# mynameisfiber/baton

Measured on NVIDIA H100. Metric: federated local samples/sec (whole box), ResNet-18 FedAvg, synthetic non-IID 32x32 shards, higher is better.
Workload: dtype bf16

## Files before the change

### baton_b200/csrc/bindings.cpp

```cpp
#include <ATen/cuda/CUDAContext.h>
#include <c10/cuda/CUDAGuard.h>
#include <torch/extension.h>

#include <optional>
#include <vector>

#include "launch.h"

namespace {

inline cudaStream_t cur_stream() { return at::cuda::getCurrentCUDAStream().stream(); }
inline void check(int rc, const char* what) {
  TORCH_CHECK(rc == 0, "baton_b200::", what, " failed with code ", rc,
              rc > 0 ? std::string(" (") + cudaGetErrorString(static_cast<cudaError_t>(rc)) + ")" : std::string());
}
inline const void* cptr(const at::Tensor& t) { return t.data_ptr(); }
inline void* ptr(at::Tensor& t) { return t.data_ptr(); }
template <class T>
inline T* opt_ptr(const std::optional<at::Tensor>& t) {
  return (t.has_value() && t->defined()) ? reinterpret_cast<T*>(t->data_ptr()) : nullptr;
}
#define CHECK_CUDA(x) TORCH_CHECK((x).is_cuda(), #x " must be a CUDA tensor")

inline std::optional<B200SgdEpilogue> sgd_epilogue(const std::optional<at::Tensor>& theta,
// ... 118 lines not shown
  return true;
}

bool conv_igemm_fwd(const at::Tensor& x, const at::Tensor& w, at::Tensor y, int64_t kh, int64_t kw, int64_t stride,
                    int64_t pad, int64_t ho, int64_t wo, int64_t cluster_k, int64_t force_bn,
                    const std::optional<at::Tensor>& col_stats) {
  CHECK_CUDA(x); CHECK_CUDA(w); CHECK_CUDA(y);
  TORCH_CHECK(x.scalar_type() == at::kBFloat16 && w.scalar_type() == at::kBFloat16 && y.scalar_type() == at::kBFloat16 &&
              x.dim() == 4 && x.is_contiguous() && w.is_contiguous() && y.is_contiguous());
  const c10::cuda::CUDAGuard guard(x.device());
  const int rc = b200_conv_igemm_fwd(cptr(x), cptr(w), ptr(y), static_cast<int>(x.size(0)), static_cast<int>(x.size(1)),
                                     static_cast<int>(x.size(2)), static_cast<int>(x.size(3)), static_cast<int>(w.size(0)),
                                     static_cast<int>(kh), static_cast<int>(kw), static_cast<int>(stride),
                                     static_cast<int>(pad), static_cast<int>(ho), static_cast<int>(wo),
                                     static_cast<int>(cluster_k), static_cast<int>(force_bn), opt_ptr<float>(col_stats),
                                     cur_stream());
  if (rc == -2) return false;
  check(rc, "conv_igemm_fwd");
  return true;
}
bool conv_igemm_dgrad(const at::Tensor& dy, const at::Tensor& w, at::Tensor dx, int64_t kh, int64_t kw, int64_t pad,
                      int64_t cluster_k, int64_t force_bn) {
  CHECK_CUDA(dy); CHECK_CUDA(w); CHECK_CUDA(dx);
  TORCH_CHECK(dy.scalar_type() == at::kBFloat16 && w.scalar_type() == at::kBFloat16 && dx.scalar_type() == at::kBFloat16 &&
              dy.dim() == 4 && dx.dim() == 4 && dy.is_contiguous() && w.is_contiguous() && dx.is_contiguous());
  const c10::cuda::CUDAGuard guard(dy.device());
  const int rc = b200_conv_igemm_dgrad(cptr(dy), cptr(w), ptr(dx), static_cast<int>(dx.size(0)), static_cast<int>(dx.size(1)),
                                       static_cast<int>(dx.size(2)), static_cast<int>(dx.size(3)), static_cast<int>(dy.size(3)),
                                       static_cast<int>(kh), static_cast<int>(kw), static_cast<int>(pad),
                                       static_cast<int>(dy.size(1)), static_cast<int>(dy.size(2)),
                                       static_cast<int>(cluster_k), static_cast<int>(force_bn), cur_stream());
  if (rc == -2) return false;
  check(rc, "conv_igemm_dgrad");
  return true;
}
bool conv_igemm_wgrad(const at::Tensor& dy, const at::Tensor& x, at::Tensor dw, int64_t cout, int64_t kh, int64_t kw,
                      int64_t stride, int64_t pad, int64_t ho, int64_t wo, int64_t split_k, int64_t force_bn,
                      const std::optional<at::Tensor>& sgd_theta, const std::optional<at::Tensor>& sgd_theta_bf16,
                      const std::optional<at::Tensor>& sgd_mom, const std::optional<at::Tensor>& sgd_hyper,
                      bool sgd_nesterov) {
  CHECK_CUDA(dy); CHECK_CUDA(x); CHECK_CUDA(dw);
  TORCH_CHECK(x.scalar_type() == at::kBFloat16 && dy.scalar_type() == at::kBFloat16 && dw.scalar_type() == at::kFloat &&
              x.dim() == 4 && x.is_contiguous() && dy.is_contiguous());
  const c10::cuda::CUDAGuard guard(x.device());
  const std::optional<B200SgdEpilogue> sgd = sgd_epilogue(sgd_theta, sgd_theta_bf16, sgd_mom, sgd_hyper, sgd_nesterov);
  const int rc = b200_conv_igemm_wgrad(cptr(dy), cptr(x), dw.data_ptr<float>(), static_cast<int>(x.size(0)),
                                       static_cast<int>(x.size(1)), static_cast<int>(x.size(2)), static_cast<int>(x.size(3)),
                                       static_cast<int>(cout), static_cast<int>(kh), static_cast<int>(kw),
                                       static_cast<int>(stride), static_cast<int>(pad), static_cast<int>(ho),
                                       static_cast<int>(wo), static_cast<int>(split_k), static_cast<int>(force_bn),
                                       sgd ? &*sgd : nullptr, cur_stream());
  if (rc == -2 || rc == B200_SGD_EPILOGUE_DECLINED) return false;
  check(rc, "conv_igemm_wgrad");
  return true;
}

void gemm_fp8(const at::Tensor& a, const at::Tensor& b, at::Tensor d, const std::optional<at::Tensor>& bias,
              const std::optional<at::Tensor>& sfa, const std::optional<at::Tensor>& sfb, int64_t M, int64_t N, int64_t K,
              int64_t lda, int64_t ldb, int64_t ldd, int64_t act, int64_t split_k, bool accumulate, double alpha) {
  CHECK_CUDA(a); CHECK_CUDA(b); CHECK_CUDA(d);
  TORCH_CHECK(a.element_size() == 1 && b.element_size() == 1, "gemm_fp8 operands must be 1-byte (e4m3)");
  const c10::cuda::CUDAGuard guard(a.device());
  check(b200_gemm_fp8(cptr(a), cptr(b), ptr(d), opt_ptr<const float>(bias), opt_ptr<const void>(sfa),
                      opt_ptr<const void>(sfb), M, N, K, lda, ldb, ldd, d.scalar_type() == at::kFloat, act, split_k,
                      accumulate, static_cast<float>(alpha), cur_stream()),
        "gemm_fp8");
// ... 405 lines not shown
                                       dw.data_ptr<float>(), opt_ptr<float>(db), loss_acc.data_ptr<float>(),
                                       opt_ptr<float>(logits_out), static_cast<int>(x.size(0)), static_cast<int>(x.size(1)),
                                       static_cast<int>(w.size(0)), static_cast<float>(grad_scale), cur_stream());
  if (rc == -2) return false;
  check(rc, "linear_xent_head");
  return true;
}
void mse(const at::Tensor& pred, const at::Tensor& target, const std::optional<at::Tensor>& dpred, at::Tensor loss_acc,
         double grad_scale) {
  CHECK_CUDA(pred);
  TORCH_CHECK(target.scalar_type() == at::kFloat && target.numel() == pred.numel());
  const c10::cuda::CUDAGuard guard(pred.device());
  const int in32 = pred.scalar_type() == at::kFloat;
  const int out32 = dpred.has_value() && dpred->defined() && dpred->scalar_type() == at::kFloat;
  check(b200_mse(pred.data_ptr(), in32, target.data_ptr<float>(), opt_ptr<void>(dpred), out32,
                 loss_acc.data_ptr<float>(), pred.numel(), static_cast<float>(grad_scale), cur_stream()),
        "mse");
}

}

PYBIND11_MODULE(TORCH_EXTENSION_NAME, m) {
  m.doc() = "baton_b200 sm_90a kernels";
  m.attr("MAX_RANKS") = B200_MAX_RANKS;
  m.def("gemm", &gemm);
  m.def("trace_set", &trace_set);
  m.def("attention_fwd", &attention_fwd);
  m.def("attention_bwd", &attention_bwd);
  m.def("bn_bwd_cluster", &bn_bwd_cluster);
  m.def("im2col_tma_probe", &im2col_tma_probe);
  m.def("conv_igemm_fwd", &conv_igemm_fwd);
  m.def("conv_igemm_wgrad", &conv_igemm_wgrad);
  m.def("conv_igemm_dgrad", &conv_igemm_dgrad);
  m.def("gemm_batched", &gemm_batched);
  m.def("gemm_fp8", &gemm_fp8);
  m.def("quant_mx_rows", &quant_mx_rows);
  m.def("quant_mx_cols", &quant_mx_cols);
  m.def("dequant_mx", &dequant_mx);
  m.def("fused_sgd", &fused_sgd);
  m.def("fused_sgd_segments", &fused_sgd_segments);
  m.def("weighted_sum", &weighted_sum);
  m.def("fold_client", &fold_client);
  m.def("cast", &cast);
  m.def("gather_rows", &gather_rows);
  m.def("colsum", &colsum);
  m.def("add_bf16", &add_bf16);
  m.def("relu_bwd", &relu_bwd);
  m.def("gelu", &gelu);
  m.def("gelu_bwd", &gelu_bwd);
  m.def("pad_rows", &pad_rows);
  m.def("embedding_bwd", &embedding_bwd);
  m.def("fedavg_allreduce", &fedavg_allreduce);
  m.def("flag_barrier", &flag_barrier);
  m.def("im2col", &im2col);
  m.def("col2im", &col2im);
  m.def("maxpool", &maxpool);
  m.def("maxpool_bwd", &maxpool_bwd);
  m.def("avgpool", &avgpool);
  m.def("avgpool_bwd", &avgpool_bwd);
  m.def("bn_stats", &bn_stats);
  m.def("bn_apply", &bn_apply);
  m.def("bn_bwd_reduce", &bn_bwd_reduce);
  m.def("bn_bwd_apply", &bn_bwd_apply);
  m.def("bn_relu_maxpool", &bn_relu_maxpool);
  m.def("bn_maxpool_bwd", &bn_maxpool_bwd);
  m.def("layernorm_fwd", &layernorm_fwd);
// ... 8 lines not shown
```

### baton_b200/csrc/gemm_wgmma.cu

```cuda
#define B200_TU_TAG 1
#include "ptx.cuh"
#include "launch.h"
#include "pdl.cuh"
#include "sgd.cuh"

namespace b200 {

constexpr int BM = 128;
constexpr int BK = 64;
constexpr int WG_K = 16;
constexpr int GEMM_THREADS = 384;
constexpr int CONSUMER_WARPS = 8;
constexpr int CONSUMER_THREADS = 32 * CONSUMER_WARPS;
constexpr int MAX_STAGES = 8;

struct GemmParams {
  int M, N, K;
  void* D;
  long long ldd;
  const float* bias;
  int out_fp32;
  int act;
  float* col_stats;
  int a_mn, b_mn;
  int k_tiles_per_split;
  int atomic_out;
  int cluster_k;
  int stages;
  const uint32_t* tile_flags;
  uint32_t flag_epoch;
  long long flag_elem_off;
  int flag_tile_elems;
  long long flag_bias_off;
  long long ldb;
  float alpha;
  int batched, batch_inner;
  int batch_count;
  long long d_outer, d_inner;
  int conv_ho, conv_wo;
  int conv_stride, conv_pad;
  int conv_kw;
  int conv_cin;
  int conv_taps;
  int conv_ncol;
  const uint32_t* flag_epoch_ptr;
  const float* sgd_hyper = nullptr;
  float* sgd_theta = nullptr;
  __nv_bfloat16* sgd_wb = nullptr;
  float* sgd_mom = nullptr;
  int sgd_nesterov = 0;
};

__device__ __forceinline__ void wait_arrival_flags(const uint32_t* flags, long long e0, long long e1, int granule,
                                                   uint32_t need) {
  for (long long t = e0 / granule; t <= e1 / granule; ++t) {
    unsigned long long spins = 0;
    while (static_cast<int32_t>(ld_acquire_sys(flags + t) - need) < 0) {
      if (++spins > (1ull << 26)) break;
    }
  }
}

template <int BN>
struct SmemLayout {
  static constexpr int A_BYTES = BM * BK * 2;
  static constexpr int B_BYTES = BN * BK * 2;
  static constexpr int STAGE_BYTES = A_BYTES + B_BYTES;
  static constexpr int PART_PITCH = BN + 4;
  static constexpr int PART_BYTES = BM * PART_PITCH * 4;
};

__device__ __forceinline__ float apply_act(float v, int act) {
  if (act == 1) return fmaxf(v, 0.f);
  if (act == 2) {
    const float k0 = 0.7978845608028654f, k1 = 0.044715f;
    float t = tanhf(k0 * (v + k1 * v * v * v));
    return 0.5f * v * (1.f + t);
  }
  return v;
}

__device__ __forceinline__ uint32_t cluster_ctarank() {
  uint32_t r;
// ... 172 lines not shown
      }
    }
  }
}

template <int BN>
__device__ __forceinline__ void consume_ktiles(float (&acc)[BN / 2], uint8_t* smem, int stages, uint64_t* full_bar,
                                               uint64_t* empty_bar, int& s, uint32_t& ph, int num_kt, int a_mn,
                                               int b_mn, int g) {
  using L = SmemLayout<BN>;
#pragma unroll
  for (int j = 0; j < BN / 2; ++j) acc[j] = 0.f;
  int prev = -1;
  for (int i = 0; i < num_kt; ++i) {
    mbar_wait(&full_bar[s], ph);
    const uint32_t sa = smem_u32(smem + s * L::STAGE_BYTES) + g * 8192;
    const uint32_t sb = smem_u32(smem + s * L::STAGE_BYTES + L::A_BYTES);
    wgmma_fence();
#pragma unroll
    for (int k = 0; k < BK / WG_K; ++k) {
      const uint64_t ad = a_mn ? gmma_desc_sw128(sa + k * 2048, 8192, 1024) : gmma_desc_sw128(sa + k * 32, 16, 1024);
      const uint64_t bd = b_mn ? gmma_desc_sw128(sb + k * 2048, 8192, 1024) : gmma_desc_sw128(sb + k * 32, 16, 1024);
      wgmma_bf16<BN>(acc, ad, bd, 1u, a_mn, b_mn);
    }
    wgmma_commit();
    wgmma_wait<1>();
    if (prev >= 0 && lane_id() == 0) mbar_arrive(&empty_bar[prev]);
    prev = s;
    if (++s == stages) { s = 0; ph ^= 1; }
  }
  wgmma_wait<0>();
  wgmma_fence_operands(acc);
  if (prev >= 0 && lane_id() == 0) mbar_arrive(&empty_bar[prev]);
}

template <int BN, int STAGES, int CONV = 0, bool SGD = false>
__global__ void __launch_bounds__(GEMM_THREADS, 1)
gemm_bf16_fixed_kernel(const __grid_constant__ CUtensorMap tmA, const __grid_constant__ CUtensorMap tmB,
                         const GemmParams p) {
  using L = SmemLayout<BN>;
  static_assert(STAGES * L::STAGE_BYTES >= L::PART_BYTES, "the drained ring must hold the fp32 accumulator tile");
  extern __shared__ __align__(1024) uint8_t smem_raw[];
  uint8_t* smem = reinterpret_cast<uint8_t*>((reinterpret_cast<uintptr_t>(smem_raw) + 1023) & ~uintptr_t(1023));
  uint64_t* full_bar = reinterpret_cast<uint64_t*>(smem + STAGES * L::STAGE_BYTES);
  uint64_t* empty_bar = full_bar + STAGES;
  float* cstat = reinterpret_cast<float*>(empty_bar + STAGES);

  griddep_launch_dependents();
  const int warp = threadIdx.x >> 5;
  const int m0 = blockIdx.y * BM;
  const int n0 = blockIdx.x * BN;
  const int k_tiles_total = (p.K + BK - 1) / BK;
  const int bz_outer = p.batched ? static_cast<int>(blockIdx.z) / p.batch_inner : 0;
  const int bz_inner = p.batched ? static_cast<int>(blockIdx.z) % p.batch_inner : 0;
  const int kt_begin = p.batched ? 0 : blockIdx.z * p.k_tiles_per_split;
  int kt_end = kt_begin + p.k_tiles_per_split;
  if (kt_end > k_tiles_total) kt_end = k_tiles_total;
  const int num_kt = kt_end - kt_begin;

  if (warp == 0 && elect_one()) {
    tma_prefetch_desc(&tmA);
    tma_prefetch_desc(&tmB);
    for (int s = 0; s < STAGES; ++s) {
      mbar_init(&full_bar[s], 1);
      mbar_init(&empty_bar[s], CONSUMER_WARPS);
    }
    fence_barrier_init();
  }
  __syncthreads();
  griddep_wait();

  if (warp == 0) {
    if (elect_one()) {
      if (p.tile_flags != nullptr) {
        const int rows_here = (p.N - n0) < BN ? (p.N - n0) : BN;
        const uint32_t need = p.flag_epoch_ptr != nullptr ? *reinterpret_cast<const volatile uint32_t*>(p.flag_epoch_ptr)
                                                          : p.flag_epoch;
        wait_arrival_flags(p.tile_flags, p.flag_elem_off + static_cast<long long>(n0) * p.ldb,
                           p.flag_elem_off + static_cast<long long>(n0 + rows_here) * p.ldb - 1, p.flag_tile_elems, need);
        if (p.flag_bias_off >= 0)
          wait_arrival_flags(p.tile_flags, p.flag_bias_off + n0, p.flag_bias_off + n0 + rows_here - 1,
                             p.flag_tile_elems, need);
        fence_proxy_async_all();
      }
      TRACE_POINT();
      for (int i = 0; i < num_kt; ++i) {
        const int s = i % STAGES;
        const uint32_t ph = (i / STAGES) & 1;
        mbar_wait(&empty_bar[s], ph ^ 1);
        uint8_t* sa = smem + s * L::STAGE_BYTES;
        uint8_t* sb = sa + L::A_BYTES;
        const int k0 = (kt_begin + i) * BK;
        if constexpr (CONV == 2) {
          const int live = (p.N - n0 + 63) / 64 < BN / 64 ? (p.N - n0 + 63) / 64 : BN / 64;
          mbar_expect_tx(&full_bar[s], L::A_BYTES + live * 8192);
        } else {
          mbar_expect_tx(&full_bar[s], L::STAGE_BYTES);
        }
        if (p.batched) {
          if (!p.a_mn) {
            tma_load_4d(sa, &tmA, &full_bar[s], k0, m0, bz_inner, bz_outer);
          } else {
#pragma unroll
            for (int j = 0; j < BM / 64; ++j)
              tma_load_4d(sa + j * 8192, &tmA, &full_bar[s], m0 + j * 64, k0, bz_inner, bz_outer);
          }
          if (!p.b_mn) {
            tma_load_4d(sb, &tmB, &full_bar[s], k0, n0, bz_inner, bz_outer);
          } else {
#pragma unroll
            for (int j = 0; j < BN / 64; ++j)
              tma_load_4d(sb + j * 8192, &tmB, &full_bar[s], n0 + j * 64, k0, bz_inner, bz_outer);
          }
        } else {
        if constexpr (CONV == 1 || CONV == 3) {
          const int kt = kt_begin + i;
          const int cblocks = p.conv_cin >> 6;
          const int tap = kt / cblocks, cb = kt - tap * cblocks;
          const int fr = tap / p.conv_kw, fs = tap - fr * p.conv_kw;
          const int q0 = m0 % p.conv_wo, t0 = m0 / p.conv_wo;
          tma_load_im2col_4d(sa, &tmA, &full_bar[s], cb * 64, q0 * p.conv_stride - p.conv_pad,
                             (t0 % p.conv_ho) * p.conv_stride - p.conv_pad, t0 / p.conv_ho, fs, fr);
        } else if (!p.a_mn) {
          tma_load_2d(sa, &tmA, &full_bar[s], k0, m0);
        } else {
#pragma unroll
          for (int j = 0; j < BM / 64; ++j)
            tma_load_2d(sa + j * 8192, &tmA, &full_bar[s], m0 + j * 64, k0);
        }
        if constexpr (CONV == 2) {
          const int q0 = k0 % p.conv_wo, t0 = k0 / p.conv_wo;
          const int w0 = q0 * p.conv_stride - p.conv_pad, h0 = (t0 % p.conv_ho) * p.conv_stride - p.conv_pad;
          const int img = t0 / p.conv_ho;
#pragma unroll
          for (int j = 0; j < BN / 64; ++j) {
            const int col = n0 + j * 64;
            if (col < p.N) {
              const int tap = col / p.conv_cin, c = col - tap * p.conv_cin;
              const int fr = tap / p.conv_kw, fs = tap - fr * p.conv_kw;
              tma_load_im2col_4d(sb + j * 8192, &tmB, &full_bar[s], c, w0, h0, img, fs, fr);
            }
          }
        } else if constexpr (CONV == 3) {
          const int kt = kt_begin + i;
          const int cblocks = p.conv_cin >> 6;
          const int tap = kt / cblocks, cb = kt - tap * cblocks;
          const int wcol = (p.conv_taps - 1 - tap) * p.conv_ncol + n0;
#pragma unroll
          for (int j = 0; j < BN / 64; ++j) tma_load_2d(sb + j * 8192, &tmB, &full_bar[s], wcol + j * 64, cb * 64);
        } else if (!p.b_mn) {
          tma_load_2d(sb, &tmB, &full_bar[s], k0, n0);
        } else {
#pragma unroll
          for (int j = 0; j < BN / 64; ++j) tma_load_2d(sb + j * 8192, &tmB, &full_bar[s], n0 + j * 64, k0);
        }
        }
      }
    }
  } else if (warp >= 4) {
    const int ew = warp - 4;
    float acc[BN / 2];
    int s = 0;
    uint32_t ph = 0;
    consume_ktiles<BN>(acc, smem, STAGES, full_bar, empty_bar, s, ph, num_kt, p.a_mn, p.b_mn, ew >> 2);
    if (threadIdx.x == 128) TRACE_POINT();
    named_bar_sync(1, CONSUMER_THREADS);
    float* part = reinterpret_cast<float*>(smem);
    wg_store_acc<BN>(acc, part, L::PART_PITCH, 64 * (ew >> 2));
    named_bar_sync(1, CONSUMER_THREADS);
    const int q = ew & 3;
    constexpr int NCHUNK = BN / 32;
    const int c_begin = (ew < 4 ? 0 : (NCHUNK + 1) / 2) * 32, c_end = (ew < 4 ? (NCHUNK + 1) / 2 : NCHUNK) * 32;
    const int lrow = q * 32 + static_cast<int>(lane_id());
    const int row = m0 + lrow;
    const bool row_ok = row < p.M;
    const size_t elt = p.out_fp32 ? 4 : 2;
    uint8_t* drow = reinterpret_cast<uint8_t*>(p.D) +
                    (static_cast<size_t>(row) * p.ldd + static_cast<size_t>(bz_outer) * p.d_outer +
                     static_cast<size_t>(bz_inner) * p.d_inner) * elt;
    const bool vec_ok = ((reinterpret_cast<uintptr_t>(p.D) & 15) == 0) && ((p.ldd * elt) % 16 == 0);
    const bool sgd_vec = SGD && (p.ldd % 4 == 0) &&
                         ((reinterpret_cast<uintptr_t>(p.sgd_theta) | reinterpret_cast<uintptr_t>(p.sgd_mom)) & 15) == 0 &&
                         (reinterpret_cast<uintptr_t>(p.sgd_wb) & 7) == 0;
    float* sstat = cstat + q * 2 * BN;
    const bool want_stats = p.col_stats != nullptr;
#pragma unroll 1
    for (int c = c_begin; c < c_end; c += 32) {
      uint32_t r[32];
      acc_ld_row32(part + lrow * L::PART_PITCH + c, r);
      const int col0 = n0 + c;
      float v[32];
#pragma unroll
      for (int j = 0; j < 32; ++j) v[j] = __uint_as_float(r[j]);
      if (col0 >= p.N) {
        if (want_stats) { sstat[c + lane_id()] = 0.f; sstat[BN + c + lane_id()] = 0.f; }
        continue;
      }
      transform_chunk<32>(p, col0, v);
      if (want_stats) stage_col_stats(sstat, BN, c, v);
      if (!row_ok) continue;
      const bool full = (col0 + 32 <= p.N);
      if constexpr (SGD) {
        sgd_epilogue_chunk(p, static_cast<size_t>(row) * p.ldd + col0, col0, v, sgd_vec);
        continue;
      }
      if (p.atomic_out) {
        float* d = reinterpret_cast<float*>(drow) + col0;
        if (full && vec_ok) {
#pragma unroll
          for (int j = 0; j < 32; j += 4)
            asm volatile("red.global.add.v4.f32 [%0], {%1, %2, %3, %4};" ::"l"(d + j), "f"(v[j]), "f"(v[j + 1]),
// ... 735 lines not shown
      (reinterpret_cast<uintptr_t>(w) & 15) || (reinterpret_cast<uintptr_t>(dx) & 15))
    return -2;
  const int bn = clamp_bn(force_bn > 0 ? force_bn : (Cin > 64 ? 128 : 64));
  CUtensorMap ta, tb;
  int rc = b200_encode_map_im2col_bf16(&ta, dy, N, Ho, Wo, Cout, KH, KW, 1, padp, 64, BM);
  if (rc) return rc;
  rc = make_map(&tb, w, Cout, static_cast<long long>(KH) * KW * Cin, static_cast<long long>(KH) * KW * Cin, 64, BK);
  if (rc) return rc;
  const int k_tiles = K / BK;
  if (cluster_k != 1 && cluster_k != 2 && cluster_k != 4 && cluster_k != 8) return -5;
  while (cluster_k > 1 && (cluster_k - 1) * ((k_tiles + cluster_k - 1) / cluster_k) >= k_tiles) cluster_k >>= 1;
  const int per = (k_tiles + cluster_k - 1) / cluster_k;
  GemmParams p;
  p.M = static_cast<int>(M); p.N = Cin; p.K = K; p.D = dx; p.ldd = Cin; p.bias = nullptr; p.out_fp32 = 0; p.act = 0;
  p.a_mn = 0; p.b_mn = 1; p.k_tiles_per_split = per; p.cluster_k = cluster_k; p.atomic_out = 0;
  p.col_stats = nullptr;
  p.tile_flags = nullptr; p.flag_epoch = 0; p.alpha = 1.0f; p.flag_elem_off = 0; p.flag_tile_elems = 0;
  p.ldb = static_cast<long long>(KH) * KW * Cin;
  p.flag_bias_off = -1; p.flag_epoch_ptr = nullptr;
  p.batched = 0; p.batch_inner = 1; p.batch_count = 1; p.d_outer = 0; p.d_inner = 0;
  const int max_stages = bn == 128 ? 6 : 8;
  p.stages = per < max_stages ? (per < 2 ? 2 : per) : max_stages;
  p.conv_ho = H; p.conv_wo = W; p.conv_stride = 1; p.conv_pad = padp; p.conv_kw = KW; p.conv_cin = Cout;
  p.conv_taps = KH * KW; p.conv_ncol = Cin;
  dim3 grid((Cin + bn - 1) / bn, static_cast<unsigned>((M + BM - 1) / BM), cluster_k);
  if (cluster_k > 1) {
    if (bn == 128) return launch_cfg<128, 3>(ta, tb, p, grid, stream);
    return launch_cfg<64, 3>(ta, tb, p, grid, stream);
  }
  if (bn == 128) return launch_fixed<128, 6, 3>(ta, tb, p, grid, stream);
  return launch_fixed<64, 8, 3>(ta, tb, p, grid, stream);
}

extern "C" int b200_conv_igemm_wgrad(const void* dy, const void* x, float* dw, int N, int H, int W, int Cin, int Cout,
                                     int KH, int KW, int stride, int pad, int Ho, int Wo, int split_k, int force_bn,
                                     const B200SgdEpilogue* sgd, cudaStream_t stream) {
  using namespace b200;
  const long long Mp = static_cast<long long>(N) * Ho * Wo;
  const int Kc = KH * KW * Cin;
  if (Mp <= 0 || Cout <= 0) return 0;
  if (Cin % 64 != 0 || Cout % 8 != 0 || Mp > (1ll << 30) || (reinterpret_cast<uintptr_t>(x) & 15) ||
      (reinterpret_cast<uintptr_t>(dy) & 15) || (reinterpret_cast<uintptr_t>(dw) & 15))
    return -2;
  const int bn = clamp_bn(force_bn > 0 ? force_bn : (Kc > 64 ? 128 : 64));
  CUtensorMap ta, tb;
  int rc = make_map(&ta, dy, Mp, Cout, Cout, 64, BK);
  if (rc) return rc;
  rc = b200_encode_map_im2col_bf16(&tb, x, N, H, W, Cin, KH, KW, stride, pad, 64, 64);
  if (rc) return rc;
  const int k_tiles = static_cast<int>((Mp + BK - 1) / BK);
  if (split_k < 1) split_k = 1;
  if (split_k > k_tiles) split_k = k_tiles;
  const int per = (k_tiles + split_k - 1) / split_k;
  split_k = (k_tiles + per - 1) / per;
  if (sgd != nullptr && split_k != 1) return B200_SGD_EPILOGUE_DECLINED;
  GemmParams p;
  if (sgd != nullptr) set_sgd_epilogue(p, *sgd);
  p.M = Cout; p.N = Kc; p.K = static_cast<int>(Mp); p.D = dw; p.ldd = Kc; p.bias = nullptr; p.out_fp32 = 1; p.act = 0;
  p.a_mn = 1; p.b_mn = 1; p.k_tiles_per_split = per; p.cluster_k = 1; p.atomic_out = 1;
  p.col_stats = nullptr;
  p.tile_flags = nullptr; p.flag_epoch = 0; p.alpha = 1.0f; p.flag_elem_off = 0; p.flag_tile_elems = 0; p.ldb = Kc;
  p.flag_bias_off = -1; p.flag_epoch_ptr = nullptr;
  p.batched = 0; p.batch_inner = 1; p.batch_count = 1; p.d_outer = 0; p.d_inner = 0;
  p.stages = 4;
  p.conv_ho = Ho; p.conv_wo = Wo; p.conv_stride = stride; p.conv_pad = pad; p.conv_kw = KW; p.conv_cin = Cin;
  p.conv_taps = KH * KW; p.conv_ncol = Cin;
// ... 11 lines not shown
```

### baton_b200/csrc/launch.h

```cpp
#pragma once
#include <cuda_runtime.h>
#include <stdint.h>

#define B200_MAX_RANKS 16

extern "C" {

struct B200SgdEpilogue {
  float* theta;
  void* theta_bf16;
  float* mom;
  const float* hyper;
  int nesterov;
};
#define B200_SGD_EPILOGUE_DECLINED (-6)

int b200_gemm_bf16(const void* a, const void* b, void* d, const float* bias, int M, int N, int K, long long lda,
                   long long ldb, long long ldd, int a_mn, int b_mn, int out_fp32, int act, int split_k, int accumulate,
                   float alpha, const uint32_t* tile_flags, uint32_t flag_epoch, long long flag_elem_off, int flag_tile_elems,
                   long long flag_bias_off, int force_bn, float* col_stats, const uint32_t* flag_epoch_ptr,
                   const B200SgdEpilogue* sgd, cudaStream_t stream);
int b200_gemm_bf16_batched(const void* a, const void* b, void* d, int M, int N, int K, long long lda, long long ldb,
                           long long ldd, int a_mn, int b_mn, int out_fp32, int act, float alpha, int n_outer,
                           int n_inner, long long a_outer, long long a_inner, long long b_outer, long long b_inner,
                           long long d_outer, long long d_inner, int accumulate, cudaStream_t stream);
int b200_attention_fwd(const void* qkv, void* out, void* probs, int B, int S, int H, int dh, float scale,
                       cudaStream_t stream);
int b200_attention_bwd(const void* qkv, const void* dout, const void* probs, void* dqkv, int B, int S, int H, int dh,
                       float scale, cudaStream_t stream);
int b200_conv_igemm_fwd(const void* x, const void* w, void* y, int N, int H, int W, int Cin, int Cout, int KH, int KW,
                        int stride, int pad, int Ho, int Wo, int cluster_k, int force_bn, float* col_stats,
                        cudaStream_t stream);
int b200_conv_igemm_dgrad(const void* dy, const void* w, void* dx, int N, int H, int W, int Cin, int Cout, int KH, int KW,
                          int pad, int Ho, int Wo, int cluster_k, int force_bn, cudaStream_t stream);
int b200_conv_igemm_wgrad(const void* dy, const void* x, float* dw, int N, int H, int W, int Cin, int Cout, int KH, int KW,
                          int stride, int pad, int Ho, int Wo, int split_k, int force_bn, const B200SgdEpilogue* sgd,
                          cudaStream_t stream);
int b200_im2col_tma_probe(const void* x, void* col, int N, int H, int W, int C, int KH, int KW, int stride, int pad,
                          int Ho, int Wo, cudaStream_t stream);
int b200_gemm_fp8(const void* a, const void* b, void* d, const float* bias, const void* sfa, const void* sfb, int M, int N,
                  int K, long long lda, long long ldb, long long ldd, int out_fp32, int act, int split_k, int accumulate,
                  float alpha, cudaStream_t stream);
int b200_quant_mx_rows(const void* x, void* q, void* sf, long long R, int C, long long ld_in, int Cp, cudaStream_t stream);
int b200_quant_mx_cols(const void* x, void* q, void* sf, long long R, int C, long long ld_in, long long Rp,
                       cudaStream_t stream);
int b200_dequant_mx(const void* q, const void* sf, float* out, long long R, int C, int Cp, cudaStream_t stream);
int b200_gemm_simt(const void* a, const void* b, void* d, const float* bias, int M, int N, int K, long long lda,
                   long long ldb, long long ldd, int a_mn, int b_mn, int out_fp32, int act, int accumulate,
                   float alpha, cudaStream_t stream);

int b200_fused_sgd(float* w, float* g, float* mom, void* w_bf16, long long n, const float* hyper, int zero_grad,
                   int nesterov, const unsigned long long* wire_slot, const float* pack_global,
                   const float* pack_scale, long long n_pack, int wire_fp32, cudaStream_t stream);
int b200_fused_sgd_segments(float* w, float* g, float* mom, void* w_bf16, const long long* segments, int n_seg,
                            const float* hyper, int nesterov, cudaStream_t stream);
int b200_fold_client(float* acc, float* theta, const float* global_w, void* w_bf16, float* mom, long long n_mom, long long n,
                     float nk, int mode, int reset, cudaStream_t stream);
int b200_weighted_sum(void* dst, const void* const* srcs, const float* weights, int n_src, long long n, int dtype,
                      cudaStream_t stream);
int b200_cast_f32_bf16(const float* src, void* dst, long long n, cudaStream_t stream);
int b200_cast_bf16_f32(const void* src, float* dst, long long n, cudaStream_t stream);
int b200_gather_rows(const void* src, const long long* idx, void* dst, long long n_rows, long long row_bytes,
                     cudaStream_t stream);
int b200_gather_rows_i64(const long long* src, const long long* idx, long long* dst, long long n,
                         cudaStream_t stream);
int b200_colsum(const void* x, float* out, long long rows, int cols, int accumulate, cudaStream_t stream);
int b200_add_bf16(const void* a, const void* b, void* out, long long n, int relu, cudaStream_t stream);
// ... 94 lines not shown
```

### baton_b200/ops/functional.py

```python
from __future__ import annotations

from typing import List, Optional, Sequence, Tuple

import torch

from ._ext import load

BF16 = torch.bfloat16
NUM_SMS = 132


def _pitch(t: torch.Tensor) -> int:
    assert t.dim() == 2 and (t.stride(1) == 1 or t.shape[1] == 1), "GEMM operand must have unit inner stride"
    return t.stride(0) if t.shape[0] > 1 else max(t.stride(0), t.shape[1])


def _tma_ok(t: torch.Tensor) -> bool:
    return t.dtype == BF16 and _pitch(t) % 8 == 0 and t.data_ptr() % 16 == 0


def pick_bn(M: int, N: int) -> int:
    m_tiles = (M + 127) // 128
    if N >= 128 and m_tiles * ((N + 127) // 128) >= NUM_SMS:
        return 128
# ... 205 lines not shown


def conv_out_size(h: int, k: int, stride: int, pad: int) -> int:
    return (h + 2 * pad - k) // stride + 1


def round_up(x: int, m: int) -> int:
    return (x + m - 1) // m * m


def im2col(x: torch.Tensor, kh: int, kw: int, stride: int, pad: int) -> Tuple[torch.Tensor, int, int, int]:
    n, h, w, c = x.shape
    ho, wo = conv_out_size(h, kh, stride, pad), conv_out_size(w, kw, stride, pad)
    kp = round_up(kh * kw * c, 8)
    col = torch.empty((n * ho * wo, kp), dtype=BF16, device=x.device)
    load().im2col(x, col, n, h, w, c, kh, kw, stride, pad, ho, wo, kp)
    return col, ho, wo, kp


def conv_igemm_fwd(x: torch.Tensor, w2d: torch.Tensor, kh: int, kw: int, stride: int, pad: int,
                   col_stats: Optional[torch.Tensor] = None) -> Optional[torch.Tensor]:
    n, h, w, c = x.shape
    cout = w2d.shape[0]
    if c % 64 or w2d.shape[1] != kh * kw * c or not x.is_contiguous() or not w2d.is_contiguous():
        return None
    ho, wo = conv_out_size(h, kh, stride, pad), conv_out_size(w, kw, stride, pad)
    M, K = n * ho * wo, kh * kw * c
    bn = pick_bn(M, cout)
    y = torch.empty((M, cout), dtype=BF16, device=x.device)
    ok = load().conv_igemm_fwd(x, w2d, y, kh, kw, stride, pad, ho, wo, pick_cluster_k(M, cout, K, bn), bn, col_stats)
    return y if ok else None


def conv_igemm_dgrad(dy: torch.Tensor, w2d: torch.Tensor, in_shape, kh: int, kw: int, pad: int) -> Optional[torch.Tensor]:
    n, h, w, c = in_shape
    cout = dy.shape[-1]
    if c % 64 or cout % 64 or w2d.shape[1] != kh * kw * c or not dy.is_contiguous() or not w2d.is_contiguous():
        return None
    M, K = n * h * w, kh * kw * cout
    bn = pick_bn(M, c)
    dx = torch.empty((n, h, w, c), dtype=BF16, device=dy.device)
    ok = load().conv_igemm_dgrad(dy, w2d, dx, kh, kw, pad, pick_cluster_k(M, c, K, bn), bn)
    return dx if ok else None


def conv_igemm_wgrad_(dy2d: torch.Tensor, x: torch.Tensor, dw2d: torch.Tensor, kh: int, kw: int, stride: int,
                      pad: int, sgd: Optional[dict] = None) -> bool:
    n, h, w, c = x.shape
    cout = dy2d.shape[1]
    if c % 64 or not x.is_contiguous() or not dy2d.is_contiguous() or not dw2d.is_contiguous():
        return False
    ho, wo = conv_out_size(h, kh, stride, pad), conv_out_size(w, kw, stride, pad)
    M, K = n * ho * wo, kh * kw * c
    bn = pick_bn(cout, K)
    split_k = pick_split_k(cout, K, M, bn)
    if sgd is not None and split_k != 1:
        return False
    sg = sgd or {}
    return bool(load().conv_igemm_wgrad(dy2d, x, dw2d, cout, kh, kw, stride, pad, ho, wo, split_k, bn,
                                        sg.get("theta"), sg.get("theta_bf16"), sg.get("momentum"), sg.get("hyper"),
                                        bool(sg.get("nesterov", False))))


def col2im(col: torch.Tensor, shape: Tuple[int, int, int, int], kh: int, kw: int, stride: int, pad: int,
           ho: int, wo: int) -> torch.Tensor:
    n, h, w, c = shape
    dx = torch.empty(shape, dtype=BF16, device=col.device)
    load().col2im(col, dx, n, h, w, c, kh, kw, stride, pad, ho, wo, col.shape[1])
    return dx


def maxpool(x: torch.Tensor, k: int, stride: int, pad: int) -> Tuple[torch.Tensor, torch.Tensor]:
    n, h, w, c = x.shape
    ho, wo = conv_out_size(h, k, stride, pad), conv_out_size(w, k, stride, pad)
    y = torch.empty((n, ho, wo, c), dtype=BF16, device=x.device)
# ... 140 lines not shown
```

### baton_b200/ops/nn.py

```python
from __future__ import annotations

import contextlib
import math
from typing import Optional

import torch
from torch import nn
from torch.nn import functional as TF

from . import functional as F
from ._ext import load

BF16 = torch.bfloat16


class _P:
    __slots__ = ("p",)

    def __init__(self, p):
        self.p = p


def _unwrap(v):
    return v.p if isinstance(v, _P) else v
# ... 296 lines not shown
        dy2 = dy.reshape(n * ho * wo, cout)
        if not dy2.is_contiguous():
            dy2 = dy2.contiguous()
        weight = ctx.weight
        k_true = kh * kw * c
        gw = None
        tgt = _grad_target(weight)
        if ctx.center:
            tap = (kh // 2) * kw + kw // 2
            if tgt is None:
                gw = torch.zeros((cout, kh, kw, c), dtype=torch.float32, device=dy.device)
                g2d = gw.view(cout, kh * kw, c)[:, tap, :]
                gw = gw.permute(0, 3, 1, 2)
            else:
                full = tgt.permute(0, 2, 3, 1).reshape(cout, kh * kw, c)
                assert full.data_ptr() == tgt.data_ptr(), "conv weight grad must be channels_last in the arena"
                g2d = full[:, tap, :]
            if tgt is None:
                F.gemm(dy2, col, a_mn=True, b_mn=True, out=g2d, accumulate=True)
            tok = WGRAD.mark(dy2)
            dx = None
            if ctx.needs_dx:
                wc = w_bf16.view(cout, kh * kw, c)[:, tap, :]
                dx = F.gemm(dy2, wc, b_mn=True).view(n, 1, 1, c)
            if tgt is not None:
                WGRAD.run(lambda: _wgrad(lambda sgd: F.gemm(dy2, col, a_mn=True, b_mn=True, out=g2d, accumulate=True,
                                                            sgd=sgd) is not None, g2d, nograd_of=tgt),
                          dy2, col, after=None if SGD_EPI.active else tok)
            return dx, gw, None, None, None, None, None, None, None, None
        igemm = getattr(ctx, "igemm", False)
        tok = WGRAD.mark(dy2)
        dx = None
        if ctx.needs_dx:
            if stride == 1 and kh == kw and kh > 1 and kp == k_true and w_bf16.shape[1] == k_true:
                dx = F.conv_igemm_dgrad(dy2.view(n, ho, wo, cout), w_bf16, (n, h, w, c), kh, kw, pad)
            if dx is None:
                dcol = F.gemm(dy2, w_bf16, b_mn=True)
                if kh == 1 and kw == 1 and stride == 1 and pad == 0 and c % 8 == 0:
                    dx = dcol.view(n, h, w, c)
                else:
                    dx = F.col2im(dcol, (n, h, w, c), kh, kw, stride, pad, ho, wo)
        if tgt is not None:
            out2d = tgt.permute(0, 2, 3, 1).reshape(cout, k_true) if tgt.dim() == 4 else tgt.view(cout, k_true)
            assert out2d.data_ptr() == tgt.data_ptr(), "conv weight grad must be channels_last in the arena"
            if igemm:
                WGRAD.run(lambda: _wgrad(lambda sgd: F.conv_igemm_wgrad_(dy2, col, out2d, kh, kw, stride, pad, sgd=sgd),
                                         out2d),
                          dy2, col, after=None if SGD_EPI.active else tok)
            else:
                WGRAD.run(lambda: F.gemm(dy2, col, a_mn=True, b_mn=True, out=out2d, accumulate=True, n_valid=k_true),
                          dy2, col, after=tok)
        elif igemm:
            g2 = torch.zeros((cout, k_true), dtype=torch.float32, device=dy.device)
            F.conv_igemm_wgrad_(dy2, col, g2, kh, kw, stride, pad)
            gw = g2.view(cout, kh, kw, c).permute(0, 3, 1, 2)
        else:
            g2 = F.gemm(dy2, col, a_mn=True, b_mn=True, out_dtype=torch.float32, accumulate=True, n_valid=k_true)
            gw = g2.view(cout, kh, kw, c).permute(0, 3, 1, 2)
        return dx, gw, None, None, None, None, None, None, None, None


class Conv2d(nn.Module):

    def __init__(self, in_channels: int, out_channels: int, kernel_size: int, stride: int = 1, padding: int = 0):
        super().__init__()
        self.in_channels, self.out_channels = in_channels, out_channels
        self.kernel_size, self.stride, self.padding = kernel_size, stride, padding
        w = torch.empty(out_channels, in_channels, kernel_size, kernel_size)
# ... 460 lines not shown
```

Baseline: 192,800.

## Add sub-pixel implicit-GEMM dgrad kernel for stride-2 convolutions

Adds a stride-2 data-gradient path that splits input pixels into four parity classes. Each class becomes an implicit GEMM over only its contributing filter taps, using im2col TMA loads of dy and a scatter epilogue into dx. It replaces the dense GEMM plus col2im fallback for stride-2 convs, avoiding both the materialised column buffer and the multiply-adds on zero-inserted positions. The cost is a new kernel mode with per-class tap tables and strided output writes, which adds complexity and correctness risk when padding and tap offsets interact.

New measurement: 198,600 (median of 6 runs). 1.03x the previous value.

```diff
diff --git a/baton_b200/csrc/bindings.cpp b/baton_b200/csrc/bindings.cpp
--- a/baton_b200/csrc/bindings.cpp
+++ b/baton_b200/csrc/bindings.cpp
@@ -174,6 +174,25 @@
                                        static_cast<int>(cluster_k), static_cast<int>(force_bn), cur_stream());
   if (rc == -2) return false;
   check(rc, "conv_igemm_dgrad");
+  return true;
+}
+bool conv_igemm_dgrad_s2(const at::Tensor& dy, const at::Tensor& w, at::Tensor dx, int64_t kh, int64_t kw,
+                         const std::vector<int64_t>& ntaps, const std::vector<int64_t>& taps, int64_t force_bn) {
+  CHECK_CUDA(dy); CHECK_CUDA(w); CHECK_CUDA(dx);
+  TORCH_CHECK(dy.scalar_type() == at::kBFloat16 && w.scalar_type() == at::kBFloat16 && dx.scalar_type() == at::kBFloat16 &&
+              dy.dim() == 4 && dx.dim() == 4 && dy.is_contiguous() && w.is_contiguous() && dx.is_contiguous());
+  TORCH_CHECK(ntaps.size() == 4 && taps.size() == 16, "conv_igemm_dgrad_s2: 4 classes x 4 taps");
+  int nt[4], tw[16];
+  for (int i = 0; i < 4; ++i) nt[i] = static_cast<int>(ntaps[i]);
+  for (int i = 0; i < 16; ++i) tw[i] = static_cast<int>(taps[i]);
+  const c10::cuda::CUDAGuard guard(dy.device());
+  const int rc = b200_conv_igemm_dgrad_s2(cptr(dy), cptr(w), ptr(dx), static_cast<int>(dx.size(0)),
+                                          static_cast<int>(dx.size(1)), static_cast<int>(dx.size(2)),
+                                          static_cast<int>(dx.size(3)), static_cast<int>(dy.size(3)), static_cast<int>(kh),
+                                          static_cast<int>(kw), static_cast<int>(dy.size(1)), static_cast<int>(dy.size(2)),
+                                          nt, tw, static_cast<int>(force_bn), cur_stream());
+  if (rc == -2) return false;
+  check(rc, "conv_igemm_dgrad_s2");
   return true;
 }
 bool conv_igemm_wgrad(const at::Tensor& dy, const at::Tensor& x, at::Tensor dw, int64_t cout, int64_t kh, int64_t kw,
@@ -645,6 +664,7 @@
   m.def("conv_igemm_fwd", &conv_igemm_fwd);
   m.def("conv_igemm_wgrad", &conv_igemm_wgrad);
   m.def("conv_igemm_dgrad", &conv_igemm_dgrad);
+  m.def("conv_igemm_dgrad_s2", &conv_igemm_dgrad_s2);
   m.def("gemm_batched", &gemm_batched);
   m.def("gemm_fp8", &gemm_fp8);
   m.def("quant_mx_rows", &quant_mx_rows);
diff --git a/baton_b200/csrc/gemm_wgmma.cu b/baton_b200/csrc/gemm_wgmma.cu
--- a/baton_b200/csrc/gemm_wgmma.cu
+++ b/baton_b200/csrc/gemm_wgmma.cu
@@ -13,6 +13,7 @@
 constexpr int CONSUMER_WARPS = 8;
 constexpr int CONSUMER_THREADS = 32 * CONSUMER_WARPS;
 constexpr int MAX_STAGES = 8;
+constexpr int S2_MAX_TAPS = 4;
 
 struct GemmParams {
   int M, N, K;
@@ -49,6 +50,9 @@
   __nv_bfloat16* sgd_wb = nullptr;
   float* sgd_mom = nullptr;
   int sgd_nesterov = 0;
+  int conv_h = 0, conv_w = 0;
+  int s2_ntaps[4] = {0, 0, 0, 0};
+  int s2_tap[4][S2_MAX_TAPS] = {};
 };
 
 __device__ __forceinline__ void wait_arrival_flags(const uint32_t* flags, long long e0, long long e1, int granule,
@@ -287,6 +291,47 @@
   wgmma_wait<0>();
   wgmma_fence_operands(acc);
   if (prev >= 0 && lane_id() == 0) mbar_arrive(&empty_bar[prev]);
+}
+
+__device__ __forceinline__ int s2_class(const GemmParams& p, int& m0) {
+  const int tiles_m = (p.M + BM - 1) / BM;
+  const int cls = static_cast<int>(blockIdx.y) / tiles_m;
+  m0 = (static_cast<int>(blockIdx.y) - cls * tiles_m) * BM;
+  return cls;
+}
+__device__ __forceinline__ int s2_ntaps(const GemmParams& p, int cls) {
+  int n = 0;
+#pragma unroll
+  for (int c = 0; c < 4; ++c) n = c == cls ? p.s2_ntaps[c] : n;
+  return n;
+}
+__device__ __forceinline__ int s2_tap(const GemmParams& p, int cls, int slot) {
+  int w = 0;
+#pragma unroll
+  for (int c = 0; c < 4; ++c)
+#pragma unroll
+    for (int t = 0; t < S2_MAX_TAPS; ++t) w = (c == cls && t == slot) ? p.s2_tap[c][t] : w;
+  return w;
+}
+__device__ __forceinline__ int s2_dx_row(const GemmParams& p, int cls, int m) {
+  if (m >= p.M) return -1;
+  const int hw = p.conv_ho * p.conv_wo;
+  const int n = m / hw, r = m - n * hw;
+  const int i = r / p.conv_wo, j = r - i * p.conv_wo;
+  const int h = 2 * i + (cls >> 1), w = 2 * j + (cls & 1);
+  return (h < p.conv_h && w < p.conv_w) ? (n * p.conv_h + h) * p.conv_w + w : -1;
+}
+template <int BN>
+__device__ __forceinline__ void s2_load_ktile(const CUtensorMap* tmA, const CUtensorMap* tmB, const GemmParams& p,
+                                              uint8_t* sa, uint8_t* sb, uint64_t* bar, int cls, int kt, int m0, int n0) {
+  const int cblocks = p.conv_cin >> 6;
+  const int slot = kt / cblocks, cb = kt - slot * cblocks;
+  const int tw = s2_tap(p, cls, slot);
+  const int q0 = m0 % p.conv_wo, t0 = m0 / p.conv_wo;
+  tma_load_im2col_4d(sa, tmA, bar, cb * 64, q0, t0 % p.conv_ho, t0 / p.conv_ho, (tw >> 24) & 0xff, (tw >> 16) & 0xff);
+  const int wcol = (tw & 0xffff) * p.conv_ncol + n0;
+#pragma unroll
+  for (int j = 0; j < BN / 64; ++j) tma_load_2d(sb + j * 8192, tmB, bar, wcol + j * 64, cb * 64);
 }
 
 template <int BN, int STAGES, int CONV = 0, bool SGD = false>
@@ -303,9 +348,10 @@
 
   griddep_launch_dependents();
   const int warp = threadIdx.x >> 5;
-  const int m0 = blockIdx.y * BM;
+  int m0 = blockIdx.y * BM;
+  const int cls = CONV == 4 ? s2_class(p, m0) : 0;
   const int n0 = blockIdx.x * BN;
-  const int k_tiles_total = (p.K + BK - 1) / BK;
+  const int k_tiles_total = CONV == 4 ? s2_ntaps(p, cls) * (p.conv_cin >> 6) : (p.K + BK - 1) / BK;
   const int bz_outer = p.batched ? static_cast<int>(blockIdx.z) / p.batch_inner : 0;
   const int bz_inner = p.batched ? static_cast<int>(blockIdx.z) % p.batch_inner : 0;
   const int kt_begin = p.batched ? 0 : blockIdx.z * p.k_tiles_per_split;
@@ -367,6 +413,8 @@
             for (int j = 0; j < BN / 64; ++j)
               tma_load_4d(sb + j * 8192, &tmB, &full_bar[s], n0 + j * 64, k0, bz_inner, bz_outer);
           }
+        } else if constexpr (CONV == 4) {
+          s2_load_ktile<BN>(&tmA, &tmB, p, sa, sb, &full_bar[s], cls, kt_begin + i, m0, n0);
         } else {
         if constexpr (CONV == 1 || CONV == 3) {
           const int kt = kt_begin + i;
@@ -428,10 +476,11 @@
     const int c_begin = (ew < 4 ? 0 : (NCHUNK + 1) / 2) * 32, c_end = (ew < 4 ? (NCHUNK + 1) / 2 : NCHUNK) * 32;
     const int lrow = q * 32 + static_cast<int>(lane_id());
     const int row = m0 + lrow;
-    const bool row_ok = row < p.M;
+    const int orow = CONV == 4 ? s2_dx_row(p, cls, row) : row;
+    const bool row_ok = CONV == 4 ? orow >= 0 : row < p.M;
     const size_t elt = p.out_fp32 ? 4 : 2;
     uint8_t* drow = reinterpret_cast<uint8_t*>(p.D) +
-                    (static_cast<size_t>(row) * p.ldd + static_cast<size_t>(bz_outer) * p.d_outer +
+                    (static_cast<size_t>(CONV == 4 && orow < 0 ? 0 : orow) * p.ldd + static_cast<size_t>(bz_outer) * p.d_outer +
                      static_cast<size_t>(bz_inner) * p.d_inner) * elt;
     const bool vec_ok = ((reinterpret_cast<uintptr_t>(p.D) & 15) == 0) && ((p.ldd * elt) % 16 == 0);
     const bool sgd_vec = SGD && (p.ldd % 4 == 0) &&
@@ -1233,6 +1282,52 @@
   return launch_fixed<64, 8, 3>(ta, tb, p, grid, stream);
 }
 
+extern "C" int b200_conv_igemm_dgrad_s2(const void* dy, const void* w, void* dx, int N, int H, int W, int Cin, int Cout,
+                                        int KH, int KW, int Ho, int Wo, const int* ntaps, const int* taps, int force_bn,
+                                        cudaStream_t stream) {
+  using namespace b200;
+  const long long M = static_cast<long long>(N) * Ho * Wo;
+  if (static_cast<long long>(N) * H * W <= 0 || Cin <= 0) return 0;
+  if (Cout % 64 != 0 || Cin % 64 != 0 || M <= 0 || static_cast<long long>(N) * H * W > (1ll << 30) ||
+      (H + 1) / 2 > Ho || (W + 1) / 2 > Wo || (reinterpret_cast<uintptr_t>(dy) & 15) ||
+      (reinterpret_cast<uintptr_t>(w) & 15) || (reinterpret_cast<uintptr_t>(dx) & 15))
+    return -2;
+  const long long tiles_m = (M + BM - 1) / BM;
+  if (4 * tiles_m > 65535) return -2;
+  GemmParams p;
+  int max_taps = 0;
+  for (int c = 0; c < 4; ++c) {
+    if (ntaps[c] < 0 || ntaps[c] > S2_MAX_TAPS) return -2;
+    for (int t = 0; t < ntaps[c]; ++t) {
+      const int tw = taps[c * S2_MAX_TAPS + t];
+      if (tw < 0 || (tw & 0xffff) >= KH * KW) return -2;
+      p.s2_tap[c][t] = tw;
+    }
+    p.s2_ntaps[c] = ntaps[c];
+    max_taps = ntaps[c] > max_taps ? ntaps[c] : max_taps;
+  }
+  if (max_taps == 0) return -2;
+  const int bn = clamp_bn(force_bn > 0 ? force_bn : (Cin > 64 ? 128 : 64));
+  CUtensorMap ta, tb;
+  int rc = b200_encode_map_im2col_bf16(&ta, dy, N, Ho, Wo, Cout, 1, 1, 1, 0, 64, BM);
+  if (rc) return rc;
+  rc = make_map(&tb, w, Cout, static_cast<long long>(KH) * KW * Cin, static_cast<long long>(KH) * KW * Cin, 64, BK);
+  if (rc) return rc;
+  const int k_tiles = max_taps * (Cout / 64);
+  p.M = static_cast<int>(M); p.N = Cin; p.K = k_tiles * BK; p.D = dx; p.ldd = Cin; p.bias = nullptr; p.out_fp32 = 0;
+  p.act = 0; p.a_mn = 0; p.b_mn = 1; p.k_tiles_per_split = k_tiles; p.cluster_k = 1; p.atomic_out = 0;
+  p.col_stats = nullptr;
+  p.tile_flags = nullptr; p.flag_epoch = 0; p.alpha = 1.0f; p.flag_elem_off = 0; p.flag_tile_elems = 0;
+  p.ldb = static_cast<long long>(KH) * KW * Cin;
+  p.flag_bias_off = -1; p.flag_epoch_ptr = nullptr;
+  p.batched = 0; p.batch_inner = 1; p.batch_count = 1; p.d_outer = 0; p.d_inner = 0;
+  p.conv_ho = Ho; p.conv_wo = Wo; p.conv_stride = 2; p.conv_pad = 0; p.conv_kw = KW; p.conv_cin = Cout;
+  p.conv_taps = KH * KW; p.conv_ncol = Cin; p.conv_h = H; p.conv_w = W;
+  dim3 grid((Cin + bn - 1) / bn, static_cast<unsigned>(4 * tiles_m), 1);
+  if (bn == 128) return launch_fixed<128, 6, 4>(ta, tb, p, grid, stream);
+  return launch_fixed<64, 8, 4>(ta, tb, p, grid, stream);
+}
+
 extern "C" int b200_conv_igemm_wgrad(const void* dy, const void* x, float* dw, int N, int H, int W, int Cin, int Cout,
                                      int KH, int KW, int stride, int pad, int Ho, int Wo, int split_k, int force_bn,
                                      const B200SgdEpilogue* sgd, cudaStream_t stream) {
diff --git a/baton_b200/csrc/launch.h b/baton_b200/csrc/launch.h
--- a/baton_b200/csrc/launch.h
+++ b/baton_b200/csrc/launch.h
@@ -33,6 +33,8 @@
                         cudaStream_t stream);
 int b200_conv_igemm_dgrad(const void* dy, const void* w, void* dx, int N, int H, int W, int Cin, int Cout, int KH, int KW,
                           int pad, int Ho, int Wo, int cluster_k, int force_bn, cudaStream_t stream);
+int b200_conv_igemm_dgrad_s2(const void* dy, const void* w, void* dx, int N, int H, int W, int Cin, int Cout, int KH,
+                             int KW, int Ho, int Wo, const int* ntaps, const int* taps, int force_bn, cudaStream_t stream);
 int b200_conv_igemm_wgrad(const void* dy, const void* x, float* dw, int N, int H, int W, int Cin, int Cout, int KH, int KW,
                           int stride, int pad, int Ho, int Wo, int split_k, int force_bn, const B200SgdEpilogue* sgd,
                           cudaStream_t stream);
diff --git a/baton_b200/ops/functional.py b/baton_b200/ops/functional.py
--- a/baton_b200/ops/functional.py
+++ b/baton_b200/ops/functional.py
@@ -261,15 +261,54 @@
     return y if ok else None
 
 
-def conv_igemm_dgrad(dy: torch.Tensor, w2d: torch.Tensor, in_shape, kh: int, kw: int, pad: int) -> Optional[torch.Tensor]:
+S2_MAX_TAPS = 4
+
+
+def conv_s2_dgrad_taps(kh: int, kw: int, pad: int, ho: int, wo: int) -> Optional[List[List[Tuple[int, int, int]]]]:
+    classes = []
+    for a in (0, 1):
+        for b in (0, 1):
+            taps = []
+            for r in range(kh):
+                if (a + pad - r) % 2:
+                    continue
+                dp = (a + pad - r) // 2
+                for s in range(kw):
+                    if (b + pad - s) % 2:
+                        continue
+                    dq = (b + pad - s) // 2
+                    if dp < 0 or dq < 0:
+                        return None
+                    if dp < ho and dq < wo:
+                        taps.append((r * kw + s, dp, dq))
+            if len(taps) > S2_MAX_TAPS:
+                return None
+            classes.append(taps)
+    return classes
+
+
+def conv_igemm_dgrad(dy: torch.Tensor, w2d: torch.Tensor, in_shape, kh: int, kw: int, pad: int, stride: int = 1,
+                     out: Optional[torch.Tensor] = None) -> Optional[torch.Tensor]:
     n, h, w, c = in_shape
     cout = dy.shape[-1]
     if c % 64 or cout % 64 or w2d.shape[1] != kh * kw * c or not dy.is_contiguous() or not w2d.is_contiguous():
         return None
-    M, K = n * h * w, kh * kw * cout
-    bn = pick_bn(M, c)
-    dx = torch.empty((n, h, w, c), dtype=BF16, device=dy.device)
-    ok = load().conv_igemm_dgrad(dy, w2d, dx, kh, kw, pad, pick_cluster_k(M, c, K, bn), bn)
+    if stride == 1:
+        M, K = n * h * w, kh * kw * cout
+        bn = pick_bn(M, c)
+        dx = out if out is not None else torch.empty((n, h, w, c), dtype=BF16, device=dy.device)
+        ok = load().conv_igemm_dgrad(dy, w2d, dx, kh, kw, pad, pick_cluster_k(M, c, K, bn), bn)
+        return dx if ok else None
+    if stride != 2:
+        return None
+    ho, wo = dy.shape[1], dy.shape[2]
+    classes = conv_s2_dgrad_taps(kh, kw, pad, ho, wo)
+    if classes is None:
+        return None
+    bn = pick_bn(4 * n * ho * wo, c)
+    words = [[t | dp << 16 | dq << 24 for t, dp, dq in taps] + [0] * (S2_MAX_TAPS - len(taps)) for taps in classes]
+    dx = out if out is not None else torch.empty((n, h, w, c), dtype=BF16, device=dy.device)
+    ok = load().conv_igemm_dgrad_s2(dy, w2d, dx, kh, kw, [len(t) for t in classes], [x for ws in words for x in ws], bn)
     return dx if ok else None
 
 
diff --git a/baton_b200/ops/nn.py b/baton_b200/ops/nn.py
--- a/baton_b200/ops/nn.py
+++ b/baton_b200/ops/nn.py
@@ -352,8 +352,8 @@
         tok = WGRAD.mark(dy2)
         dx = None
         if ctx.needs_dx:
-            if stride == 1 and kh == kw and kh > 1 and kp == k_true and w_bf16.shape[1] == k_true:
-                dx = F.conv_igemm_dgrad(dy2.view(n, ho, wo, cout), w_bf16, (n, h, w, c), kh, kw, pad)
+            if kp == k_true and w_bf16.shape[1] == k_true and (stride == 2 or (stride == 1 and kh == kw and kh > 1)):
+                dx = F.conv_igemm_dgrad(dy2.view(n, ho, wo, cout), w_bf16, (n, h, w, c), kh, kw, pad, stride=stride)
             if dx is None:
                 dcol = F.gemm(dy2, w_bf16, b_mn=True)
                 if kh == 1 and kw == 1 and stride == 1 and pad == 0 and c % 8 == 0:
```
